# zero-savvy/vimz

Measured on AMD Instinct MI355X. Metric: nova_folding_steps_per_sec, higher is better.
Workload: dtype u32 limbs (256-bit Montgomery integers over BN254 Fr/Fq)

## Files before the change

vimz_amd/csrc/capi.hip:

```cpp
#include <hip/hip_runtime.h>
#include <mutex>
#include <new>
#include <string>
#include <cstring>
#include <cstdio>

#include "internal.hpp"
#define HIP_TRY(c, x) do { hipError_t _e = (x); if (_e != hipSuccess) return vz::vz_fail(c, VIMZ_ERR_HIP, #x, _e); } while (0)
#include "vecops_api.hpp"
#include "ckgen.hpp"

using namespace vz;

static thread_local std::string g_err_noctx;

namespace vz {
int vz_fail(vimz_ctx* c, int code, const char* what, hipError_t e) {
  std::string m = what;
  if (e != hipSuccess) { m += ": "; m += hipGetErrorString(e); }
  static std::mutex err_mu;
  std::lock_guard<std::mutex> g(err_mu);
  if (c) c->err = m; else g_err_noctx = m;
  return code;
}
// ... 601 lines not shown
  uint64_t total = 0;
  for (size_t k = 0; k < blocks; k++) for (size_t g = 0; g < nb; g++) { sum[g] += block_hist[k * nb + g]; total += block_hist[k * nb + g]; }
  if (total >= (1ull << 31)) return fail(c, VIMZ_ERR_INVALID, "vimz_test_msm_scan: more than 2^31 - 1 entries");
  std::lock_guard<std::mutex> g(c->mu);
  HIP_TRY(c, hipSetDevice(c->device));
  TailBufs B;
  uint32_t *hist, *counts, *boff, *soff, *totals, *heavy;
  const size_t heavy_words = 1 + (size_t)MSM_HEAVY_CAP + TAIL_HEAVY_GUARD;
  TAIL_TRY(B.get(&hist, blocks * nb)); TAIL_TRY(B.get(&counts, nb)); TAIL_TRY(B.get(&boff, nb + 1, 0xff)); TAIL_TRY(B.get(&soff, nb + 1, 0xff));
  TAIL_TRY(B.get(&totals, MSM_TOTALS_WORDS, 0)); TAIL_TRY(B.get(&heavy, heavy_words, 0xff));
  for (int call = 0; call < calls; call++) {
    if (lds) {
      TAIL_TRY(tail_up(c, hist, block_hist, blocks * nb));
      launch_prefix_scan(c->stream, hist, (uint32_t)nb, counts, (uint32_t)blocks, heavy, boff, soff, totals, sub, heavy_min, MsmRowStrides(), 1);
    } else {
      TAIL_TRY(tail_up(c, counts, sum.data(), nb));
      TAIL_TRY(hipMemsetAsync(heavy, 0, 4, c->stream));
      launch_scan(c->stream, counts, (uint32_t)nb, boff, soff, totals, sub, heavy, heavy_min);
    }
    TAIL_TRY(hipGetLastError());
    TAIL_TRY(hipStreamSynchronize(c->stream));
  }
  TAIL_TRY(tail_down(c, counts_out, counts, nb)); TAIL_TRY(tail_down(c, bucket_off_out, boff, nb + 1)); TAIL_TRY(tail_down(c, sub_off_out, soff, nb + 1));
  TAIL_TRY(tail_down(c, totals_out, totals, 4)); TAIL_TRY(tail_down(c, heavy_out, heavy, heavy_words));
  if (lds) TAIL_TRY(tail_down(c, block_hist_out, hist, blocks * nb));
  TAIL_TRY(hipStreamSynchronize(c->stream));
  return VIMZ_OK;
}

extern "C" int vimz_test_msm_combine(vimz_ctx* c, int curve, uint32_t* partial, size_t n_slots, const uint32_t* sub_off, size_t nb, const uint32_t* heavy, size_t n_ids, int lane_bits,
                                     uint32_t heavy_min, size_t rows, int calls) {
  if (!c || !partial || !sub_off || !heavy || calls < 1 || !nb || nb >= (1u << 24) || n_slots >= (1u << 24)) return fail(c, VIMZ_ERR_INVALID, "vimz_test_msm_combine: bad argument");
  if (curve < VIMZ_CURVE_BN254_G1 || curve > VIMZ_CURVE_VESTA) return fail(c, VIMZ_ERR_INVALID, "vimz_test_msm_combine: bad curve");
  if (lane_bits < 0 || lane_bits > 4) return fail(c, VIMZ_ERR_INVALID, "vimz_test_msm_combine: lane_bits outside 0..4");
  if (!rows || rows > MSM_ROWS_MAX) return fail(c, VIMZ_ERR_INVALID, "vimz_test_msm_combine: rows outside 1..16");
  if (n_ids > MSM_HEAVY_CAP) return fail(c, VIMZ_ERR_INVALID, "vimz_test_msm_combine: more ids than the heavy list holds");
  for (size_t r = 0; r < rows; r++) {
    const uint32_t* off = sub_off + r * (nb + 1); const uint32_t* hv = heavy + r * (1 + n_ids);
    if (!tail_offsets_ok(off, nb, n_slots)) return fail(c, VIMZ_ERR_INVALID, "vimz_test_msm_combine: sub_off not monotone or outside partial");
    if (hv[0] > MSM_HEAVY_CAP) continue;
    if (hv[0] > n_ids) return fail(c, VIMZ_ERR_INVALID, "vimz_test_msm_combine: the heavy count exceeds the ids given");
    std::vector<bool> seen(nb, false);
    for (uint32_t h = 0; h < hv[0]; h++) {
      const uint32_t b = hv[1 + h];
      if (b >= nb) return fail(c, VIMZ_ERR_INVALID, "vimz_test_msm_combine: a heavy bucket id not below nb");
      if (seen[b] || off[b + 1] - off[b] <= heavy_min) return fail(c, VIMZ_ERR_INVALID, "vimz_test_msm_combine: a heavy bucket listed twice or not above heavy_min");
      seen[b] = true;
    }
  }
  std::lock_guard<std::mutex> g(c->mu);
  HIP_TRY(c, hipSetDevice(c->device));
  const uint32_t G = (uint32_t)rows;
  const MsmRowStrides rs = msm_row_strides(G, 0, (uint32_t)nb, 0, n_slots, 0);
  TailBufs B;
  uint32_t *dp, *doff, *dheavy, *dscr, *ddone;
  TAIL_TRY(B.get(&dp, rows * XYZZ_WORDS * n_slots)); TAIL_TRY(B.get(&doff, rows * (nb + 1))); TAIL_TRY(B.get(&dheavy, rows * ((size_t)MSM_HEAVY_CAP + 1), 0xff));
  TAIL_TRY(B.get(&dscr, rows * MsmWorkspace::HEAVY_SCRATCH_WORDS, 0xff)); TAIL_TRY(B.get(&ddone, rows * (size_t)MSM_HEAVY_DONE_WORDS, 0));
  TAIL_TRY(tail_up(c, doff, sub_off, rows * (nb + 1)));
  for (size_t r = 0; r < rows; r++) TAIL_TRY(tail_up(c, dheavy + r * ((size_t)MSM_HEAVY_CAP + 1), heavy + r * (1 + n_ids), 1 + n_ids));
  const int rc = curve_dispatch(curve, [&](auto cv) {
    typedef typename decltype(cv)::Coord F;
    for (int call = 0; call < calls; call++) {
      TAIL_TRY(tail_up(c, dp, partial, rows * XYZZ_WORDS * n_slots));
      launch_combine<F>(c->stream, dp, doff, (uint32_t)nb, dheavy, dscr, (uint32_t)lane_bits, heavy_min, ddone, rs, G);
      TAIL_TRY(hipGetLastError());
      TAIL_TRY(hipStreamSynchronize(c->stream));
    }
    return (int)VIMZ_OK;
  });
  if (rc) return rc;
  TAIL_TRY(tail_down(c, partial, dp, rows * XYZZ_WORDS * n_slots));
  TAIL_TRY(hipStreamSynchronize(c->stream));
  return VIMZ_OK;
}

extern "C" int vimz_test_msm_reduce(vimz_ctx* c, int curve, const uint32_t* partial, size_t n_slots, const uint32_t* counts, const uint32_t* sub_off, uint32_t nbw, size_t windows,
                                    int mode, size_t rows, int calls, uint32_t* sums_out) {
  if (!c || !partial || !counts || !sub_off || !sums_out || calls < 1 || mode < 0 || mode > 2 || n_slots >= (1u << 24)) return fail(c, VIMZ_ERR_INVALID, "vimz_test_msm_reduce: bad argument");
  if (curve < VIMZ_CURVE_BN254_G1 || curve > VIMZ_CURVE_VESTA) return fail(c, VIMZ_ERR_INVALID, "vimz_test_msm_reduce: bad curve");
  if (nbw < 2 || nbw > 32768 || (nbw & (nbw - 1))) return fail(c, VIMZ_ERR_INVALID, "vimz_test_msm_reduce: nbw not a power of two in 2..32768");
  if (!rows || rows > MSM_ROWS_MAX) return fail(c, VIMZ_ERR_INVALID, "vimz_test_msm_reduce: rows outside 1..16");
  uint32_t Pl = 0, Gp = 0;
  const bool planes_fit = msm_plane_shape(nbw, Pl, Gp);
  if (!windows || windows > (size_t)MSM_MAX_WINDOWS / 2 || (mode == 2 && (windows != 1 || rows != 1 || !planes_fit)))
    return fail(c, VIMZ_ERR_INVALID, "vimz_test_msm_reduce: windows outside 1..48, or bit planes over anything but one row of one bucket set of 1024 buckets or more");
  const size_t nb = (size_t)nbw * windows;
  for (size_t r = 0; r < rows; r++) {
    const uint32_t* off = sub_off + r * (nb + 1);
    if (!tail_offsets_ok(off, nb, n_slots)) return fail(c, VIMZ_ERR_INVALID, "vimz_test_msm_reduce: sub_off not monotone or outside partial");
    for (size_t b = 0; b < nb; b++) if (counts[r * nb + b] && off[b] >= n_slots) return fail(c, VIMZ_ERR_INVALID, "vimz_test_msm_reduce: a filled bucket's slot outside partial");
  }
  std::lock_guard<std::mutex> g(c->mu);
  HIP_TRY(c, hipSetDevice(c->device));
  const uint32_t G = (uint32_t)rows;
  const size_t kout = mode == 2 ? Pl + 2 : mode == 1 ? 2 * windows : windows;
  const MsmRowStrides rs = msm_row_strides(G, 0, (uint32_t)nb, 0, n_slots, (size_t)XYZZ_WORDS * kout);
  TailBufs B;
// ... 315 lines not shown
```

vimz_amd/csrc/ec.hpp:

```cpp
#pragma once
#include "fp.hpp"
#include "fp29.hpp"

namespace vz {

template <class F>
struct Affine { F x, y; };

template <class F>
struct XYZZ {
  F X, Y, ZZ, ZZZ;
  static VZ_HD XYZZ identity() { XYZZ r; r.X = F::zero(); r.Y = F::zero(); r.ZZ = F::zero(); r.ZZZ = F::zero(); return r; }
  VZ_HD bool is_identity() const { return ZZ.is_zero(); }
};

template <class F>
VZ_HD bool aff_is_identity(const Affine<F>& a) { return a.x.is_zero() && a.y.is_zero(); }

template <class F>
VZ_HD XYZZ<F> from_affine(const Affine<F>& a) {
  XYZZ<F> r;
  if (aff_is_identity(a)) return XYZZ<F>::identity();
  r.X = a.x; r.Y = a.y; r.ZZ = F::one(); r.ZZZ = F::one();
  return r;
}


template <class F>
VZ_HD XYZZ<F> dbl_affine(const Affine<F>& a) {
  XYZZ<F> r;
  F U = F::dbl(a.y);
  F V = F::sqr(U);
  F W = F::mul(U, V);
  F S = F::mul(a.x, V);
  F X2 = F::sqr(a.x);
  F M = F::add(F::dbl(X2), X2);
  r.X = F::template sub<4>(F::sqr(M), F::dbl(S));
  r.Y = F::template sub<2>(F::mul(M, F::template sub<6>(S, r.X)), F::mul(W, a.y));
  r.ZZ = V; r.ZZZ = W;
  return r;
}

template <class F>
VZ_HD XYZZ<F> dbl(const XYZZ<F>& p) {
  if (p.is_identity()) return p;
  XYZZ<F> r;
  F U = F::dbl(p.Y);
  F V = F::sqr(U);
  F W = F::mul(U, V);
  F S = F::mul(p.X, V);
  F X2 = F::sqr(p.X);
  F M = F::add(F::dbl(X2), X2);
  r.X = F::template sub<4>(F::sqr(M), F::dbl(S));
  r.Y = F::template sub<2>(F::mul(M, F::template sub<6>(S, r.X)), F::mul(W, p.Y));
  r.ZZ = F::mul(V, p.ZZ);
  r.ZZZ = F::mul(W, p.ZZZ);
  return r;
}

template <int K, class F>
VZ_HD F diff_of_products(const F& a, const F& b, const F& c, const F& d) {
  if constexpr (F::LAZY) return F::mul_add2(a, b, F::template sub<K>(F::zero(), c), d);
  else return F::template sub<2>(F::mul(a, b), F::mul(c, d));
}

template <class F>
VZ_HD void add_mixed(XYZZ<F>& acc, const Affine<F>& q) {
  if (aff_is_identity(q)) return;
  if (acc.is_identity()) { acc.X = q.x; acc.Y = q.y; acc.ZZ = F::one(); acc.ZZZ = F::one(); return; }
  F U2 = F::mul(q.x, acc.ZZ);
  F S2 = F::mul(q.y, acc.ZZZ);
  F Pv = F::template sub<6>(U2, acc.X);
  F R = F::template sub<4>(S2, acc.Y);
  if (Pv.is_zero_mod()) {
    if (R.is_zero_mod()) acc = dbl_affine(q); else acc = XYZZ<F>::identity();
    return;
  }
  F PP = F::sqr(Pv);
  F PPP = F::mul(Pv, PP);
  F Q = F::mul(acc.X, PP);
  F X3 = F::template sub<4>(F::sqr(R), F::add(PPP, F::dbl(Q)));
  F Y3 = diff_of_products<4>(R, F::template sub<6>(Q, X3), acc.Y, PPP);
  acc.X = X3; acc.Y = Y3;
  acc.ZZ = F::mul(acc.ZZ, PP);
  acc.ZZZ = F::mul(acc.ZZZ, PPP);
}

template <class F>
VZ_HD void add_full(XYZZ<F>& acc, const XYZZ<F>& q) {
  if (q.is_identity()) return;
  if (acc.is_identity()) { acc = q; return; }
  F U1 = F::mul(acc.X, q.ZZ);
  F U2 = F::mul(q.X, acc.ZZ);
  F S1 = F::mul(acc.Y, q.ZZZ);
  F S2 = F::mul(q.Y, acc.ZZZ);
  F Pv = F::template sub<2>(U2, U1);
  F R = F::template sub<2>(S2, S1);
  if (Pv.is_zero_mod()) {
    if (R.is_zero_mod()) acc = dbl(acc); else acc = XYZZ<F>::identity();
    return;
  }
  F PP = F::sqr(Pv);
  F PPP = F::mul(Pv, PP);
  F Q = F::mul(U1, PP);
  F X3 = F::template sub<4>(F::sqr(R), F::add(PPP, F::dbl(Q)));
  F Y3 = diff_of_products<2>(R, F::template sub<6>(Q, X3), S1, PPP);
  acc.X = X3; acc.Y = Y3;
  acc.ZZ = F::mul(F::mul(acc.ZZ, q.ZZ), PP);
  acc.ZZZ = F::mul(F::mul(acc.ZZZ, q.ZZZ), PPP);
}

template <class F>
VZ_HD Affine<F> to_affine(const XYZZ<F>& p) {
  Affine<F> a;
  if (p.is_identity()) { a.x = F::zero(); a.y = F::zero(); return a; }
  F zi3 = F::pow_pm2(p.ZZZ);
  F zi2 = F::sqr(F::mul(zi3, p.ZZ));
  a.x = F::mul(p.X, zi2).canon();
// ... 31 lines not shown
```

vimz_amd/csrc/msm.hpp:

```cpp
#pragma once
#include <cstdlib>
#include <cstring>
#include <mutex>
#include "msm_api.hpp"
#include "ec_mem.hpp"

namespace vz {

inline const MsmTuning& msm_tuning() {
  static const MsmTuning t = [] {
    MsmTuning r;
    if (const char* e = getenv("VIMZ_TUNE")) {
      if (const char* q = strstr(e, "sort_blocks=")) r.sort_blocks = atoi(q + 12);
      if (const char* q = strstr(e, "combine_lane_bits=")) r.combine_lane_bits = atoi(q + 18);
      if (const char* q = strstr(e, "ones_dense=")) r.ones_dense = atoi(q + 11);
      if (const char* q = strstr(e, "reduce_planes=")) r.reduce_planes = atoi(q + 14);
      if (const char* q = strstr(e, "signed_scalars=")) r.signed_scalars = atoi(q + 15) != 0;
    }
    return r;
  }();
  return t;
}


__device__ __forceinline__ uint32_t window_bits(const uint32_t* s, int lo, int c) {
  int limb = lo >> 5, off = lo & 31;
  if (limb >= 8) return 0;
  uint64_t v = s[limb];
  if (limb + 1 < 8) v |= (uint64_t)s[limb + 1] << 32;
  return (uint32_t)(v >> off) & ((1u << c) - 1);
}

template <class S>
__device__ __forceinline__ bool load_scalar(const uint32_t* __restrict__ scalars, size_t i, int mont, int skip_ones, int sgn, uint32_t* s, uint32_t& flip) {
  const uint4* p = reinterpret_cast<const uint4*>(scalars + 8 * i);
  uint4 a = p[0], b = p[1];
  S x;
  x.v[0] = a.x; x.v[1] = a.y; x.v[2] = a.z; x.v[3] = a.w; x.v[4] = b.x; x.v[5] = b.y; x.v[6] = b.z; x.v[7] = b.w;
  if (x.is_zero()) return false;
  if (skip_ones) {
    bool one;
    if (mont) one = x.eq(S::one());
    else { uint32_t o = x.v[0] ^ 1u; for (int k = 1; k < 8; k++) o |= x.v[k]; one = o == 0; }
    if (one) return false;
  }
  if (mont) x = S::from_mont(x);
  flip = 0;
  if (sgn) {
    uint32_t t[8]; uint64_t br = 0, lt = 0;
#pragma unroll
// ... 167 lines not shown
  const uint32_t* mine = block_hist + (size_t)blockIdx.x * nb;
  for (uint32_t g = threadIdx.x; g < nb; g += SORT_THREADS) lds_pos[g] = bucket_off[g] + mine[g];
  __syncthreads();
  const size_t chunk = (n + gridDim.x - 1) / gridDim.x;
  const size_t lo = blockIdx.x * chunk, hi = lo + chunk < n ? lo + chunk : n;
  for (size_t i = lo + threadIdx.x; i < hi; i += SORT_THREADS) {
    uint32_t s[8], flip;
    if (!load_scalar<S>(scalars, i, mont, skip_ones, sgn, s, flip)) continue;
    for_each_digit(s, c, K, flip, [&](int w, uint32_t b, uint32_t neg) {
      const uint32_t pos = atomicAdd(&lds_pos[(uint32_t)w * nbw + b], 1u);
      sorted[pos] = ((uint32_t)i + (uint32_t)w * pt_stride) | (neg << 31);
    });
  }
}

template <class F>
__global__ void __launch_bounds__(256, 3) k_accum(const uint32_t* __restrict__ bases, const uint32_t* __restrict__ sorted,
                                               const uint32_t* __restrict__ bucket_off, const uint32_t* __restrict__ sub_off,
                                               uint32_t nb, const uint32_t* __restrict__ totals,
                                               uint32_t* __restrict__ partial, uint32_t sub, MsmRowStrides rs) {
  { const size_t row = blockIdx.y; sorted += row * rs.sorted; bucket_off += row * rs.offs; sub_off += row * rs.offs; totals += row * rs.totals; partial += row * rs.partial; }
  const uint32_t total = totals[0];
  uint32_t s = blockIdx.x * blockDim.x + threadIdx.x;
  if (s >= total) return;
  uint32_t lo = 0, hi = nb;
  while (hi - lo > 1) {
    uint32_t mid = (lo + hi) >> 1;
    if (sub_off[mid] <= s) lo = mid; else hi = mid;
  }
  const uint32_t b = lo, k = s - sub_off[b];
  const uint32_t beg = bucket_off[b] + k * sub;
  const uint32_t end = min(bucket_off[b + 1], beg + sub);
  XYZZ<F> acc = XYZZ<F>::identity();
  uint32_t ent = beg < end ? sorted[beg] : 0u;
  RawAffine raw = load_affine_raw(bases, ent & 0x7fffffffu);
  for (uint32_t e = beg; e < end; e++) {
    const uint32_t ent_n = e + 1 < end ? sorted[e + 1] : ent;
    const RawAffine raw_n = load_affine_raw(bases, ent_n & 0x7fffffffu);
    Affine<F> q = affine_of_raw<F>(raw);
    if ((ent >> 31) && !aff_is_identity(q)) q.y = F::neg(q.y);
    add_mixed(acc, q);
    ent = ent_n; raw = raw_n;
  }
  store_xyzz(partial, s, acc);
}

constexpr uint32_t ONES_THREADS = 16384;
template <class S>
__device__ __forceinline__ bool scalar_is_one(const uint32_t* __restrict__ scalars, size_t i, int mont) {
  const uint4* p = reinterpret_cast<const uint4*>(scalars + 8 * i);
  const uint4 a = p[0], b = p[1];
  if (mont) return a.x == S::Params::R1.w[0] && a.y == S::Params::R1.w[1] && a.z == S::Params::R1.w[2] && a.w == S::Params::R1.w[3] &&
                   b.x == S::Params::R1.w[4] && b.y == S::Params::R1.w[5] && b.z == S::Params::R1.w[6] && b.w == S::Params::R1.w[7];
  return a.x == 1u && (a.y | a.z | a.w | b.x | b.y | b.z | b.w) == 0u;
}
template <class S, class F>
__global__ void __launch_bounds__(256) k_ones_partial(const uint32_t* __restrict__ scalars, const uint32_t* __restrict__ bases, size_t n, int mont,
                                                      uint32_t* __restrict__ out ) {
  const uint32_t t = blockIdx.x * blockDim.x + threadIdx.x;
  XYZZ<F> acc = XYZZ<F>::identity();
  for (size_t i = t; i < n; i += ONES_THREADS)
    if (scalar_is_one<S>(scalars, i, mont)) { Affine<F> q = load_affine<F>(bases, (uint32_t)i); add_mixed(acc, q); }
  store_xyzz(out, t, acc);
}
template <class S, class F>
__device__ __forceinline__ XYZZ<F> ones_dense_sum(const uint32_t* __restrict__ scalars, const uint32_t* __restrict__ bases, size_t n, int mont, uint32_t (*queue)[128]) {
  const uint32_t t = blockIdx.x * blockDim.x + threadIdx.x, lane = threadIdx.x & 63u, wv = threadIdx.x >> 6;
  const size_t wave = t >> 6, nwaves = ONES_THREADS / 64;
  volatile uint32_t* q = queue[wv];
  XYZZ<F> acc = XYZZ<F>::identity();
  uint32_t cnt = 0;
  for (size_t base = wave * 64; base < n; base += nwaves * 64) {
    const size_t i = base + lane;
    const bool one = i < n && scalar_is_one<S>(scalars, i, mont);
    const uint64_t m = __ballot(one);
    if (one) q[cnt + (uint32_t)__popcll(m & ((1ull << lane) - 1ull))] = (uint32_t)i;
    cnt += (uint32_t)__popcll(m);
    __builtin_amdgcn_wave_barrier();
    if (cnt >= 64) {
      cnt -= 64;
      const uint32_t idx = q[cnt + lane];
      __builtin_amdgcn_wave_barrier();
      Affine<F> pt = load_affine<F>(bases, idx);
      add_mixed(acc, pt);
    }
  }
  if (lane < cnt) { Affine<F> pt = load_affine<F>(bases, q[lane]); add_mixed(acc, pt); }
  return acc;
}
template <class S, class F>
__global__ void __launch_bounds__(256) k_ones_dense(const uint32_t* __restrict__ scalars, const uint32_t* __restrict__ bases, size_t n, int mont,
                                                    uint32_t* __restrict__ out ) {
  __shared__ uint32_t queue[4][128];
  const XYZZ<F> acc = ones_dense_sum<S, F>(scalars, bases, n, mont, queue);
  store_xyzz(out, blockIdx.x * blockDim.x + threadIdx.x, acc);
}
template <class S, class F>
__global__ void __launch_bounds__(256) k_ones_dense_rows(OnesDescs ds, int mont, uint32_t* __restrict__ lvl ) {
  __shared__ uint32_t queue[4][128];
  __shared__ XYZZ<F> sh[256];
  const OnesDesc& d = ds.d[blockIdx.y];
  sh[threadIdx.x] = ones_dense_sum<S, F>(d.scalars, d.bases, d.n, mont, queue);
  __syncthreads();
  quad_tree256<F>(sh);
  if (threadIdx.x == 0) store_xyzz(lvl, (size_t)blockIdx.y * gridDim.x + blockIdx.x, sh[0]);
}
template <class F>
__global__ void __launch_bounds__(256) k_tree_rows(const uint32_t* __restrict__ lvl, uint32_t m , OnesDescs ds) {
  __shared__ XYZZ<F> sh[256];
  const uint32_t t = threadIdx.x;
  sh[t] = t < m ? load_xyzz<F>(lvl, (size_t)blockIdx.x * m + t) : XYZZ<F>::identity();
  __syncthreads();
  quad_tree256<F>(sh);
  if (t == 0) store_xyzz(ds.d[blockIdx.x].out, 0, sh[0]);
}
template <class F>
__global__ void __launch_bounds__(256) k_tree256(const uint32_t* __restrict__ in, uint32_t m, uint32_t* __restrict__ out) {
  __shared__ XYZZ<F> sh[256];
  const uint32_t t = threadIdx.x, i = blockIdx.x * 256 + t;
  sh[t] = i < m ? load_xyzz<F>(in, i) : XYZZ<F>::identity();
  __syncthreads();
  quad_tree256<F>(sh);
  if (t == 0) store_xyzz(out, blockIdx.x, sh[0]);
}


constexpr uint32_t MSM_HEAVY_PARTS = 32, MSM_HEAVY_SPLIT = 1024;
constexpr uint32_t MSM_HEAVY_SPLIT_MIN = 2048;
constexpr uint32_t COMBINE_HEAVY_BLOCKS = 512, COMBINE_SPLIT_BLOCKS = 1024;

template <class F>
__global__ void __launch_bounds__(256) k_combine(uint32_t* __restrict__ partial, const uint32_t* __restrict__ sub_off, uint32_t nb, uint32_t nbn,
                                                 const uint32_t* __restrict__ heavy, uint32_t heavy_cap, uint32_t* scratch ,
                                                 uint32_t lane_bits , uint32_t heavy_min,
                                                 uint32_t* __restrict__ heavy_done , MsmRowStrides rs) {
  __shared__ XYZZ<F> sh[256];
  __shared__ uint32_t s_last;
  const uint32_t t = threadIdx.x;
  { const size_t row = blockIdx.y; partial += row * rs.partial; sub_off += row * rs.offs; heavy += row * rs.heavy; scratch += row * rs.heavy_scratch; heavy_done += row * rs.heavy_done; }
  if (blockIdx.x < nbn) {
    const uint32_t L = 1u << lane_bits, lane = t & (L - 1u);
    const uint32_t b = blockIdx.x * (256u >> lane_bits) + (t >> lane_bits);
    uint32_t s0 = 0, m = 0;
    if (b < nb) { s0 = sub_off[b]; m = sub_off[b + 1] - s0; }
    if (m > heavy_min && heavy[0] <= heavy_cap) m = 0;
    if (!__syncthreads_or(m >= 2 ? 1 : 0)) return;
    XYZZ<F> acc = XYZZ<F>::identity();
    if (lane < m) acc = load_xyzz<F>(partial, s0 + lane);
    for (uint32_t k = lane + L; k < m; k += L) { XYZZ<F> q = load_xyzz<F>(partial, s0 + k); add_full(acc, q); }
    sh[t] = acc;
    __syncthreads();
    for (uint32_t d = L >> 1; d > 0; d >>= 1) {
      if (lane < d && lane + d < m) { XYZZ<F> a = sh[t]; add_full(a, sh[t + d]); sh[t] = a; }
      __syncthreads();
    }
    if (lane == 0 && m >= 2) store_xyzz(partial, s0, sh[t]);
    return;
  }
  const uint32_t count = heavy[0] <= heavy_cap ? heavy[0] : 0u;
  if (blockIdx.x < nbn + COMBINE_HEAVY_BLOCKS) {
    for (uint32_t h = blockIdx.x - nbn; h < count; h += COMBINE_HEAVY_BLOCKS) {
      const uint32_t b = heavy[1 + h];
      const uint32_t s0 = sub_off[b], m = sub_off[b + 1] - s0;
      if (h < MSM_HEAVY_SPLIT && m >= MSM_HEAVY_SPLIT_MIN) continue;
      XYZZ<F> acc = XYZZ<F>::identity();
      for (uint32_t k = t; k < m; k += 256) { XYZZ<F> q = load_xyzz<F>(partial, s0 + k); add_full(acc, q); }
      __syncthreads();
      sh[t] = acc;
      __syncthreads();
      quad_tree256<F>(sh);
      if (t == 0) store_xyzz(partial, s0, sh[0]);
    }
// ... 164 lines not shown
        if (dig[k]) atomicAdd(&cnt[(dig[k] < 0 ? -dig[k] : dig[k]) - 1], 1u);
      }
    }
  }
  __syncthreads();
  if (t < 64) {
    const uint32_t c0 = cnt[t];
    uint32_t m4 = (c0 + 3) / 4, m5 = (c0 + 4) / 5, m6 = (c0 + 5) / 6, m7 = (c0 + 6) / 7;
    for (int o = 32; o > 0; o >>= 1) { m4 += __shfl_xor(m4, o); m5 += __shfl_xor(m5, o); m6 += __shfl_xor(m6, o); m7 += __shfl_xor(m7, o); }
    const uint32_t sub = m4 <= SMALL_THREADS ? 4u : m5 <= SMALL_THREADS ? 5u : m6 <= SMALL_THREADS ? 6u : m7 <= SMALL_THREADS ? 7u : 8u;
    const uint32_t m = (c0 + sub - 1) / sub;
    uint32_t ic = c0, im = m, mx = m;
    for (int o = 1; o < 64; o <<= 1) {
      const uint32_t uc = __shfl_up(ic, o), um = __shfl_up(im, o);
      if ((int)t >= o) { ic += uc; im += um; }
    }
    for (int o = 32; o > 0; o >>= 1) mx = max(mx, (uint32_t)__shfl_xor(mx, o));
    off[t] = ic - c0; soff[t] = im - m;
    if (t == 63) { off[SMALL_NBW] = ic; soff[SMALL_NBW] = im; s_maxm = mx; }
  }
  __syncthreads();
#pragma unroll
  for (int k = 0; k < (int)SMALL_PER_THREAD; k++) {
    if (dig[k]) {
      const uint32_t b = (uint32_t)(dig[k] < 0 ? -dig[k] : dig[k]) - 1;
      const uint32_t pos = atomicAdd(&cur[b], 1u);
      list[off[b] + pos] = (uint16_t)((t + SMALL_THREADS * k) | (dig[k] < 0 ? 0x8000u : 0u));
    }
  }
  if (t < SMALL_NBW) for (uint32_t sb = soff[t]; sb < soff[t + 1]; sb++) subb[sb] = (uint8_t)t;
  __syncthreads();
  const uint32_t nsubs = soff[SMALL_NBW];
  XYZZ<F> acc = XYZZ<F>::identity();
  uint32_t kk = 0, mb = 0;
  if (t < nsubs) {
    const uint32_t b = subb[t];
    kk = t - soff[b]; mb = soff[b + 1] - soff[b];
    const uint32_t cb = off[b + 1] - off[b];
    const uint32_t beg = off[b] + kk * cb / mb, end = off[b] + (kk + 1) * cb / mb;
    uint32_t ent = beg < end ? list[beg] : 0u;
    Affine<F> pt = load_affine<F>(wbases, lo + (ent & 0x7fffu));
    for (uint32_t e = beg; e < end; e++) {
      const uint32_t ent_n = e + 1 < end ? list[e + 1] : ent;
      const Affine<F> pt_n = load_affine<F>(wbases, lo + (ent_n & 0x7fffu));
      if ((ent & 0x8000u) && !aff_is_identity(pt)) pt.y = F::neg(pt.y);
      add_mixed(acc, pt);
      ent = ent_n; pt = pt_n;
    }
  }
  sh[t] = acc;
  __syncthreads();
  for (uint32_t d = 1; d < s_maxm; d <<= 1) {
    const bool act = t < nsubs && (kk & (2 * d - 1)) == 0 && kk + d < mb;
    const uint64_t bal = __ballot(act);
    if ((t & 63) == 0) wcnt[t >> 6] = (uint32_t)__popcll(bal);
    __syncthreads();
    uint32_t before = 0, total = 0;
    for (uint32_t wv = 0; wv < SMALL_THREADS / 64; wv++) { before += wv < (t >> 6) ? wcnt[wv] : 0u; total += wcnt[wv]; }
    if (act) list[before + (uint32_t)__popcll(bal & ((1ull << (t & 63)) - 1ull))] = (uint16_t)t;
    __syncthreads();
    for (uint32_t base = 0; base < total; base += 64)
      quad_level<F>(sh, min(64u, total - base), [&](uint32_t e) { return (uint32_t)list[base + e]; }, [&](uint32_t e) { return (uint32_t)list[base + e] + d; });
  }
  XYZZ<F> bk = XYZZ<F>::identity();
  if (t < SMALL_NBW && cnt[t]) bk = sh[soff[t]];
  __syncthreads();
  if (Q > 1 && done) {
    if (t < SMALL_NBW) {
      store_xyzz(chunk_out, ((size_t)w * Q + q) * SMALL_NBW + t, bk);
      __threadfence();
      if (t == 0) s_ticket = atomicAdd(&done[w], 1u);
    }
    __syncthreads();
    if (s_ticket != Q - 1) return;
    __threadfence();

    const uint32_t b = t & (SMALL_NBW - 1), sl = t / SMALL_NBW;
    for (uint32_t loaded = 0; loaded < Q;) {
      const uint32_t slot0 = loaded ? 1u : 0u, k = min(Q - loaded, 4u - slot0), m = slot0 + k;
// ... 138 lines not shown
    for (int k = 0; k < c; k++) acc = dbl(acc);
    p = to_affine(acc);
    store_affine<F>(tables, (size_t)j * n + i, p);
  }
}
template <class C>
hipError_t build_tables(hipStream_t stream, const uint32_t* d_bases, size_t n, int c, int K, uint32_t* d_tables) {
  typedef typename C::Coord F;
  if (!n) return hipSuccess;
  hipLaunchKernelGGL(k_build_tables<F>, dim3((unsigned)((n + 255) / 256)), dim3(256), 0, stream, d_bases, n, c, K, d_tables);
  return hipGetLastError();
}

static inline MsmRowStrides msm_row_strides(uint32_t G, size_t scalar_words, uint32_t nb, size_t entries, size_t max_subs, size_t out_words) {
  MsmRowStrides rs;
  if (G > 1) {
    rs.scalars = scalar_words; rs.block_hist = (size_t)SORT_BLOCKS * nb; rs.sorted = entries; rs.partial = (size_t)XYZZ_WORDS * max_subs;
    rs.heavy_scratch = MsmWorkspace::HEAVY_SCRATCH_WORDS; rs.out = out_words;
    rs.counts = nb; rs.offs = nb + 1; rs.totals = MSM_TOTALS_WORDS; rs.heavy = MSM_HEAVY_CAP + 1; rs.heavy_done = MSM_HEAVY_DONE_WORDS;
  }
  return rs;
}
static inline void launch_prefix_scan(hipStream_t stream, uint32_t* block_hist, uint32_t nb, uint32_t* counts, uint32_t sort_blocks, uint32_t* heavy, uint32_t* bucket_off,
                                      uint32_t* sub_off, uint32_t* totals, uint32_t sub, uint32_t heavy_min, const MsmRowStrides& rs, uint32_t G) {
  hipLaunchKernelGGL(k_prefix_scan<0>, dim3((nb + 1023) / 1024, G), dim3(1024), 0, stream, block_hist, nb, counts, sort_blocks, heavy, bucket_off, sub_off,
                     totals, sub, heavy_min, MSM_HEAVY_CAP, rs);
}
static inline void launch_scan(hipStream_t stream, const uint32_t* counts, uint32_t nb, uint32_t* bucket_off, uint32_t* sub_off, uint32_t* totals, uint32_t sub, uint32_t* heavy,
                               uint32_t heavy_min) {
  hipLaunchKernelGGL(k_scan<MSM_SUB>, dim3(1), dim3(1024), 0, stream, counts, nb, bucket_off, sub_off, totals, sub, heavy, heavy_min, MSM_HEAVY_CAP);
}
template <class F>
static void launch_combine(hipStream_t stream, uint32_t* partial, const uint32_t* sub_off, uint32_t nb, const uint32_t* heavy, uint32_t* heavy_scratch, uint32_t lane_bits,
                           uint32_t heavy_min, uint32_t* heavy_done, const MsmRowStrides& rs, uint32_t G) {
  const unsigned per_wg = 256u >> lane_bits, nbn = (nb + per_wg - 1) / per_wg;
  hipLaunchKernelGGL(k_combine<F>, dim3(nbn + COMBINE_HEAVY_BLOCKS + COMBINE_SPLIT_BLOCKS, G), dim3(256), 0, stream, partial, sub_off, nb, nbn,
                     heavy, MSM_HEAVY_CAP, heavy_scratch, lane_bits, heavy_min, heavy_done, rs);
}
template <class F>
static void launch_reduce(hipStream_t stream, const uint32_t* partial, const uint32_t* counts, const uint32_t* sub_off, uint32_t nbw, uint32_t windows, uint32_t* window_sums,
                          uint32_t* plain_sums, const MsmRowStrides& rs, uint32_t G) {
  hipLaunchKernelGGL(k_reduce<F>, dim3(windows, G), dim3(nbw < 256 ? nbw : 256), 0, stream, partial, counts, sub_off, nbw, window_sums, plain_sums, rs);
}
template <class F>
static void launch_reduce_planes(hipStream_t stream, const uint32_t* partial, const uint32_t* counts, const uint32_t* sub_off, uint32_t nbw, uint32_t Pl, uint32_t Gp,
                                 uint32_t* plane_scratch, uint32_t* ticket, uint32_t* out) {
  hipLaunchKernelGGL(k_reduce_planes<F>, dim3((Pl + 2) * Gp), dim3(256), 0, stream, partial, counts, sub_off, nbw, Pl, Gp, nbw / (512u * Gp), plane_scratch, ticket, out);
}
template <class F>
static void launch_accum(hipStream_t stream, const uint32_t* bases, const uint32_t* sorted, const uint32_t* bucket_off, const uint32_t* sub_off, uint32_t nb, const uint32_t* totals,
                         uint32_t* partial, uint32_t sub, size_t max_subs, const MsmRowStrides& rs, uint32_t G) {
  hipLaunchKernelGGL(k_accum<F>, dim3((unsigned)((max_subs + 255) / 256), G), dim3(256), 0, stream, bases, sorted, bucket_off, sub_off, nb, totals, partial, sub, rs);
}
template <class S, class F>
static void launch_ones(hipStream_t stream, bool dense, const uint32_t* scalars, const uint32_t* bases, size_t n, int mont, uint32_t* lvl0) {
  if (dense) hipLaunchKernelGGL((k_ones_dense<S, F>), dim3(ONES_THREADS / 256), dim3(256), 0, stream, scalars, bases, n, mont, lvl0);
  else hipLaunchKernelGGL((k_ones_partial<S, F>), dim3(ONES_THREADS / 256), dim3(256), 0, stream, scalars, bases, n, mont, lvl0);
}
template <class F>
static void launch_tree256(hipStream_t stream, const uint32_t* in, uint32_t m, uint32_t* tmp, uint32_t* out) {
  if (m > 256) {
    hipLaunchKernelGGL(k_tree256<F>, dim3((m + 255) / 256), dim3(256), 0, stream, in, m, tmp);
    in = tmp; m = (m + 255) / 256;
  }
  hipLaunchKernelGGL(k_tree256<F>, dim3(1), dim3(256), 0, stream, in, m, out);
}
template <class F>
static void launch_tree_rows(hipStream_t stream, const uint32_t* lvl, uint32_t m, const OnesDescs& ds, uint32_t count) {
  hipLaunchKernelGGL(k_tree_rows<F>, dim3(count), dim3(256), 0, stream, lvl, m, ds);
}
// ... 96 lines not shown

template <class C>
static hipError_t launch_unit_sums(const MsmCall& a, const MsmShape& sh, uint32_t G) {
  typedef typename C::Coord F;
  typedef typename C::Scalar S;
  const MsmRowGroup* rg = a.rg;
  if (rg) {
    OnesDesc ds[2 * MSM_ROWS_MAX];
    for (uint32_t r = 0; r < G; r++) ds[r] = OnesDesc{a.d_scalars + 8 * r * rg->scalar_row_stride, a.d_bases, a.wsum + r * (rg->pinned_row_stride / 4) + (size_t)XYZZ_WORDS * sh.kout, a.n};
    for (uint32_t e = 0; e < rg->n_extra; e++) ds[G + e] = rg->extra[e];
    return ones_launch_rows<C>(a.stream, a.ws, ds, G + rg->n_extra, a.scalars_mont);
  }
  uint32_t* lvl0 = reinterpret_cast<uint32_t*>(a.ws.ones_partial);
  launch_ones<S, F>(a.stream, msm_tuning().ones_dense != 0, a.d_scalars, a.d_bases, a.n, a.scalars_mont, lvl0);
  uint32_t* lvl1 = lvl0 + (size_t)XYZZ_WORDS * ONES_THREADS;
  launch_tree256<F>(a.stream, lvl0, ONES_THREADS, lvl1, a.wsum + (size_t)XYZZ_WORDS * sh.kout);
  return hipSuccess;
}

template <class C>
static hipError_t launch_large(const MsmCall& a, const MsmShape& sh) {
  typedef typename C::Coord F;
  typedef typename C::Scalar S;
  const MsmPlan& pl = sh.plan;
  const MsmRowGroup* rg = a.rg;
  MsmWorkspace& ws = a.ws;
  const uint32_t G = rg ? rg->G : 1u;
  VZ_HIP_CHECK(ws.reserve(pl.nb, sh.entries, sh.max_subs, rg ? std::max<size_t>(G, rg->max_rows) : 1));
  const MsmRowStrides rs = msm_row_strides(G, rg ? 8 * rg->scalar_row_stride : 0, pl.nb, sh.entries, sh.max_subs, rg ? rg->pinned_row_stride / 4 : 0);
  VZ_HIP_CHECK(launch_sort<S>(a, sh, rs, G));
  uint32_t* partial = reinterpret_cast<uint32_t*>(ws.partial);
  launch_accum<F>(a.stream, a.d_bases, ws.sorted, ws.bucket_off, ws.sub_off, pl.nb, ws.totals, partial, sh.sub, sh.max_subs, rs, G);
  VZ_EV(4);
  launch_combine<F>(a.stream, partial, ws.sub_off, pl.nb, ws.heavy, ws.heavy_scratch, sh.lane_bits, sh.heavy_min, ws.heavy_done, rs, G);
  VZ_EV(5);
  if (sh.planes) launch_reduce_planes<F>(a.stream, partial, ws.counts, ws.sub_off, pl.nbw, sh.Pl, sh.Gp, ws.plane_scratch, ws.totals + 3, a.wsum);
  else if (sh.shared) launch_reduce<F>(a.stream, partial, ws.counts, ws.sub_off, sh.vw, (uint32_t)sh.V, a.wsum, a.wsum + (size_t)XYZZ_WORDS * sh.V, rs, G);
  else launch_reduce<F>(a.stream, partial, ws.counts, ws.sub_off, pl.nbw, (uint32_t)pl.K, a.wsum, nullptr, rs, G);
  VZ_EV(6);
  if (a.split_ones) VZ_HIP_CHECK(launch_unit_sums<C>(a, sh, G));
  return hipGetLastError();
}
#undef VZ_EV

template <class C>
static hipError_t msm_launch_impl(hipStream_t stream, MsmWorkspace& ws, const uint32_t* d_bases, const uint32_t* d_scalars, size_t n,
                                  int scalars_mont, int c_override, void* pinned_dst, MsmPlan* plan_out, hipEvent_t* ev, int split_ones,
                                  const BaseTables* tb, const MsmRowGroup* rg) {
  MsmShape sh;
  MsmGroupDesc gd;
  if (rg) { gd.grouped = true; gd.G = rg->G; gd.n_extra = rg->n_extra; }
  const int rc = msm_shape(sh, n, C::Scalar::Params::BITS, c_override, split_ones, msm_table_desc(tb), gd, msm_tuning(), msm_no_small());
  if (rc != MSM_SHAPE_OK) return rc == MSM_SHAPE_NOT_SUPPORTED ? hipErrorNotSupported : hipErrorInvalidValue;
  *plan_out = sh.plan;
  if (sh.path == MSM_PATH_LARGE && sh.plan.tabled) d_bases = tb->d + (size_t)AFFINE_WORDS * tb->offset;
  const MsmCall a{stream, ws, d_bases, d_scalars, n, scalars_mont, msm_tuning().signed_scalars, split_ones, reinterpret_cast<uint32_t*>(pinned_dst), ev, tb, rg};
  switch (sh.path) {
    case MSM_PATH_FIXED: return launch_fixed<C>(a, sh);
    case MSM_PATH_SMALL: return launch_small<C>(a, sh, msm_small_sum_kernel());
    default: return launch_large<C>(a, sh);
  }
}

template <class C>
hipError_t msm_launch(hipStream_t stream, MsmWorkspace& ws, const uint32_t* d_bases, const uint32_t* d_scalars, size_t n,
                      int scalars_mont, int c_override, void* pinned_dst, MsmPlan* plan_out, hipEvent_t* ev, int split_ones,
                      const BaseTables* tb) {
// ... 113 lines not shown
```

vimz_amd/csrc/msm_shape.hpp:

```cpp
#pragma once
#include <cstdint>
#include <cstddef>
#include <algorithm>

namespace vz {

constexpr int MSM_SUB = 16;
constexpr int MSM_MAX_WINDOWS = 96;
constexpr uint32_t MSM_VWIN = 1024;
constexpr uint32_t MSM_ROWS_MAX = 16;

struct MsmPlan {
  int c;
  int K;
  uint32_t nbw;
  uint32_t nb;
  int split_ones;
  int tabled;
};

constexpr int SMALL_C = 7;
constexpr uint32_t SMALL_CHUNK = 1536, SMALL_MAXQ = 32;
constexpr uint32_t SMALL_NBW = 1u << (SMALL_C - 1);
constexpr size_t MSM_SMALL_MAX = (size_t)SMALL_CHUNK * 20;
static_assert(MSM_SMALL_MAX <= (size_t)SMALL_CHUNK * SMALL_MAXQ, "chunk results of a window fit the workspace");
constexpr uint32_t FIXED_PER_THREAD = 4, FIXED_CHUNK = 256 * FIXED_PER_THREAD;
constexpr uint32_t SORT_BLOCKS = 256;
constexpr uint32_t MSM_TOTALS_WORDS = 16, MSM_HEAVY_CAP = 65536, MSM_HEAVY_DONE_WORDS = 1024;
constexpr uint32_t MSM_HEAVY_SCRATCH_POINTS = 1024 * 32;

static inline MsmPlan msm_plan(size_t n, int scalar_bits, int c_override) {
  MsmPlan p;
  p.split_ones = 0; p.tabled = 0;
  int c = c_override;
  if (c <= 0) {
    c = n >= (1u << 15) ? 11 : n >= (1u << 12) ? 9 : n >= 256 ? 7 : 5;
  }
  p.c = c;
  p.K = (scalar_bits + 1 + c - 1) / c;
  p.nbw = 1u << (c - 1);
  p.nb = p.nbw * (uint32_t)p.K;
  return p;
}

static inline uint32_t msm_vwin(const MsmPlan& p) { return std::min<uint32_t>(p.nbw, MSM_VWIN); }
static inline int msm_vwindows(const MsmPlan& p) { return (int)(p.nbw / msm_vwin(p)); }
static inline uint32_t msm_plane_bits(const MsmPlan& p) { uint32_t P = 0; while ((1u << P) < p.nbw) P++; return P; }
static inline bool msm_plane_shape(uint32_t nbw, uint32_t& Pl, uint32_t& Gp) {
  Pl = 0; while ((1u << Pl) < nbw) Pl++;
  Gp = std::min<uint32_t>(16u, nbw / 1024u);
  while (Gp > 1 && (Pl + 2) * Gp > 256) Gp >>= 1;
  return nbw >= 1024 && (1u << Pl) == nbw && (Pl + 2) * Gp <= 256 && (int)Pl + 2 + 1 <= MSM_MAX_WINDOWS;
}
static inline int msm_kout(const MsmPlan& p) { return p.tabled == 4 ? (int)msm_plane_bits(p) + 2 : p.tabled == 1 ? 2 * msm_vwindows(p) : p.K; }
static inline int msm_sums_out(const MsmPlan& p) { return msm_kout(p) + (p.split_ones ? 1 : 0); }

struct MsmTuning { int sort_blocks = 0, combine_lane_bits = -1, ones_dense = 1, reduce_planes = 0, signed_scalars = 1; };
struct MsmTableDesc { bool present = false; int c = 0, K = 0, own = 0; bool mult = false; size_t n_total = 0; };
struct MsmGroupDesc { bool grouped = false; uint32_t G = 1, n_extra = 0; };

enum MsmPath { MSM_PATH_FIXED, MSM_PATH_SMALL, MSM_PATH_LARGE };
enum { MSM_SHAPE_OK = 0, MSM_SHAPE_INVALID = 1, MSM_SHAPE_NOT_SUPPORTED = 2  };

struct MsmShape {
  MsmPath path = MSM_PATH_LARGE;
  MsmPlan plan = {};
  uint32_t Q = 0, chunk = 0, Qf = 0;
  bool lds_sort = false;
  bool own = false;
  bool shared = false;
  bool planes = false;
  uint32_t sub = 0;
  size_t entries = 0, max_subs = 0;
  uint32_t sort_blocks = 0, lane_bits = 0, heavy_min = 0;
  uint32_t bstride = 0 , pstride = 0 ;
  uint32_t vw = 0; int V = 0;
  uint32_t Pl = 0, Gp = 0;
  int kout = 0;
};

static inline int msm_shape(MsmShape& out, size_t n, int scalar_bits, int c_override, int split_ones, const MsmTableDesc& tb, const MsmGroupDesc& rg,
                            const MsmTuning& tune, bool no_small) {
  MsmShape s;
  if (n == 0 || n >= (1u << 31)) return MSM_SHAPE_INVALID;
  if (rg.grouped && (rg.G == 0 || rg.G > MSM_ROWS_MAX || rg.n_extra > MSM_ROWS_MAX || (split_ones == 0 && rg.n_extra))) return MSM_SHAPE_INVALID;
  const bool small_fmt = tb.present && tb.c == SMALL_C;
  const bool small_tb = small_fmt && !no_small && c_override <= 0;
  bool tabled = tb.present && !small_fmt && c_override <= 0;
  if (tabled && tb.own && tb.c != msm_plan(n, scalar_bits, 0).c) tabled = false;
  s.own = tabled && tb.own;
  s.shared = tabled && !tb.own;
  if (small_tb && (n > MSM_SMALL_MAX || tb.K != (scalar_bits + SMALL_C) / SMALL_C)) return MSM_SHAPE_INVALID;
  if (!no_small && !tabled && c_override <= 0 && n <= MSM_SMALL_MAX) {
    if (rg.grouped) return MSM_SHAPE_NOT_SUPPORTED;
    MsmPlan& ps = s.plan;
    ps.c = SMALL_C; ps.K = (scalar_bits + SMALL_C) / SMALL_C; ps.nbw = SMALL_NBW; ps.nb = SMALL_NBW * (uint32_t)ps.K; ps.split_ones = 0; ps.tabled = small_tb ? 2 : 0;
    s.kout = msm_kout(ps);
    if (small_tb && tb.mult) {
      s.path = MSM_PATH_FIXED;
      s.Qf = (uint32_t)((n + FIXED_CHUNK - 1) / FIXED_CHUNK);
    } else {
      s.path = MSM_PATH_SMALL;
      s.Q = (uint32_t)((n + SMALL_CHUNK - 1) / SMALL_CHUNK); s.chunk = (uint32_t)((n + s.Q - 1) / s.Q);
    }
    out = s;
    return MSM_SHAPE_OK;
  }
  s.path = MSM_PATH_LARGE;
  MsmPlan& pl = s.plan;
  pl = msm_plan(n, scalar_bits, tabled ? tb.c : c_override);
  if (tabled) {
    if (tb.K != pl.K || pl.nbw < 256 || (size_t)tb.K * tb.n_total >= (1u << 31)) return MSM_SHAPE_INVALID;
    if (!s.own && 2 * msm_vwindows(pl) + 1 > MSM_MAX_WINDOWS) return MSM_SHAPE_INVALID;
    if (s.own) pl.tabled = 3; else { pl.nb = pl.nbw; pl.tabled = 1; }
  }
  if (pl.K + 1 > MSM_MAX_WINDOWS || pl.c > 16 || pl.c < 2) return MSM_SHAPE_INVALID;
  pl.split_ones = split_ones;
  const bool planes_fit = msm_plane_shape(pl.nbw, s.Pl, s.Gp);
  s.planes = s.shared && tune.reduce_planes && planes_fit;
  if (s.planes) pl.tabled = 4;
  s.lds_sort = (size_t)pl.nb * 4 <= 144 * 1024;
  if (rg.grouped && (s.planes || s.own || !s.lds_sort)) return MSM_SHAPE_NOT_SUPPORTED;
  s.entries = (size_t)pl.K * n;
  s.sub = n < (1u << 15) ? 8u : split_ones ? (n < (1u << 19) ? 8u : (uint32_t)MSM_SUB) : (uint32_t)MSM_SUB;
  s.max_subs = s.entries / s.sub + pl.nb + 1;
  s.sort_blocks = tune.sort_blocks > 0 && tune.sort_blocks <= (int)SORT_BLOCKS ? (uint32_t)tune.sort_blocks
                                                                                 : (uint32_t)std::min<size_t>(SORT_BLOCKS, std::max<size_t>(32, n / 4096));
  s.bstride = s.shared ? 0u : pl.nbw; s.pstride = tabled ? (uint32_t)tb.n_total : 0u;
  const size_t mean_parts = (split_ones ? s.entries / 8 : s.entries) / s.sub / pl.nb + 1;
  s.lane_bits = tune.combine_lane_bits >= 0 ? (uint32_t)tune.combine_lane_bits : mean_parts > 96 ? 4u : mean_parts > 48 ? 3u : mean_parts > 24 ? 2u : 1u;
  s.heavy_min = 16u << s.lane_bits;
  s.vw = msm_vwin(pl); s.V = msm_vwindows(pl); s.kout = msm_kout(pl);
  out = s;
  return MSM_SHAPE_OK;
}

}
```

Before: 1430.

## Add packed slot-parallel MSM combine and cheaper first mixed addition

Adds a packed combine mode that assigns one thread per partial-sum slot across all buckets and runs a workgroup tree reduction in LDS with compacted pair lists. The old mode mapped a fixed number of lanes to each bucket. The packed mode is on by default when heavy_min is at most 32, and it is meant to avoid idle lanes when buckets hold few partials. Separately, the first mixed addition after an affine load now skips the ZZ/ZZZ multiplies (add_mixed_first), and dbl_affine gains a y==0 identity check. The costs are a larger shared-memory array, which may lower occupancy, and extra barriers per reduction level.

```diff
diff --git a/vimz_amd/csrc/capi.hip b/vimz_amd/csrc/capi.hip
--- a/vimz_amd/csrc/capi.hip
+++ b/vimz_amd/csrc/capi.hip
@@ -657,6 +657,8 @@
                                      uint32_t heavy_min, size_t rows, int calls) {
   if (!c || !partial || !sub_off || !heavy || calls < 1 || !nb || nb >= (1u << 24) || n_slots >= (1u << 24)) return fail(c, VIMZ_ERR_INVALID, "vimz_test_msm_combine: bad argument");
   if (curve < VIMZ_CURVE_BN254_G1 || curve > VIMZ_CURVE_VESTA) return fail(c, VIMZ_ERR_INVALID, "vimz_test_msm_combine: bad curve");
+  const bool packed = lane_bits >= 0 && (lane_bits & 0x100) != 0;
+  if (packed) lane_bits &= 0xff;
   if (lane_bits < 0 || lane_bits > 4) return fail(c, VIMZ_ERR_INVALID, "vimz_test_msm_combine: lane_bits outside 0..4");
   if (!rows || rows > MSM_ROWS_MAX) return fail(c, VIMZ_ERR_INVALID, "vimz_test_msm_combine: rows outside 1..16");
   if (n_ids > MSM_HEAVY_CAP) return fail(c, VIMZ_ERR_INVALID, "vimz_test_msm_combine: more ids than the heavy list holds");
@@ -687,7 +689,7 @@
     typedef typename decltype(cv)::Coord F;
     for (int call = 0; call < calls; call++) {
       TAIL_TRY(tail_up(c, dp, partial, rows * XYZZ_WORDS * n_slots));
-      launch_combine<F>(c->stream, dp, doff, (uint32_t)nb, dheavy, dscr, (uint32_t)lane_bits, heavy_min, ddone, rs, G);
+      launch_combine<F>(c->stream, dp, doff, (uint32_t)nb, dheavy, dscr, (uint32_t)lane_bits, heavy_min, ddone, rs, G, packed, n_slots);
       TAIL_TRY(hipGetLastError());
       TAIL_TRY(hipStreamSynchronize(c->stream));
     }
diff --git a/vimz_amd/csrc/ec.hpp b/vimz_amd/csrc/ec.hpp
--- a/vimz_amd/csrc/ec.hpp
+++ b/vimz_amd/csrc/ec.hpp
@@ -28,6 +28,7 @@
 
 template <class F>
 VZ_HD XYZZ<F> dbl_affine(const Affine<F>& a) {
+  if (a.y.is_zero_mod()) return XYZZ<F>::identity();
   XYZZ<F> r;
   F U = F::dbl(a.y);
   F V = F::sqr(U);
@@ -84,6 +85,34 @@
   acc.X = X3; acc.Y = Y3;
   acc.ZZ = F::mul(acc.ZZ, PP);
   acc.ZZZ = F::mul(acc.ZZZ, PPP);
+}
+
+template <class F>
+VZ_HD void add_mixed_first(XYZZ<F>& acc, const Affine<F>& q) {
+  if (aff_is_identity(q)) return;
+  if (acc.is_identity()) { acc.X = q.x; acc.Y = q.y; acc.ZZ = F::one(); acc.ZZZ = F::one(); return; }
+  F Pv = F::template sub<2>(q.x, acc.X);
+  F R = F::template sub<2>(q.y, acc.Y);
+  if (Pv.is_zero_mod()) {
+    if (R.is_zero_mod()) acc = dbl_affine(q); else acc = XYZZ<F>::identity();
+    return;
+  }
+  F PP = F::sqr(Pv);
+  F PPP = F::mul(Pv, PP);
+  F Q = F::mul(acc.X, PP);
+  F X3 = F::template sub<4>(F::sqr(R), F::add(PPP, F::dbl(Q)));
+  F Y3 = diff_of_products<2>(R, F::template sub<6>(Q, X3), acc.Y, PPP);
+  acc.X = X3; acc.Y = Y3;
+  acc.ZZ = PP;
+  acc.ZZZ = PPP;
+}
+
+template <class F>
+VZ_HD void add_mixed_chain(XYZZ<F>& acc, bool& plain, const Affine<F>& q) {
+  if (aff_is_identity(q)) return;
+  if (acc.is_identity()) { acc.X = q.x; acc.Y = q.y; acc.ZZ = F::one(); acc.ZZZ = F::one(); plain = true; return; }
+  if (plain) { add_mixed_first(acc, q); plain = false; }
+  else add_mixed(acc, q);
 }
 
 template <class F>
diff --git a/vimz_amd/csrc/msm.hpp b/vimz_amd/csrc/msm.hpp
--- a/vimz_amd/csrc/msm.hpp
+++ b/vimz_amd/csrc/msm.hpp
@@ -16,6 +16,7 @@
       if (const char* q = strstr(e, "ones_dense=")) r.ones_dense = atoi(q + 11);
       if (const char* q = strstr(e, "reduce_planes=")) r.reduce_planes = atoi(q + 14);
       if (const char* q = strstr(e, "signed_scalars=")) r.signed_scalars = atoi(q + 15) != 0;
+      if (const char* q = strstr(e, "combine_packed=")) r.combine_packed = atoi(q + 15) != 0;
     }
     return r;
   }();
@@ -249,6 +250,7 @@
   const uint32_t beg = bucket_off[b] + k * sub;
   const uint32_t end = min(bucket_off[b + 1], beg + sub);
   XYZZ<F> acc = XYZZ<F>::identity();
+  bool plain = false;
   uint32_t ent = beg < end ? sorted[beg] : 0u;
   RawAffine raw = load_affine_raw(bases, ent & 0x7fffffffu);
   for (uint32_t e = beg; e < end; e++) {
@@ -256,7 +258,7 @@
     const RawAffine raw_n = load_affine_raw(bases, ent_n & 0x7fffffffu);
     Affine<F> q = affine_of_raw<F>(raw);
     if ((ent >> 31) && !aff_is_identity(q)) q.y = F::neg(q.y);
-    add_mixed(acc, q);
+    add_mixed_chain(acc, plain, q);
     ent = ent_n; raw = raw_n;
   }
   store_xyzz(partial, s, acc);
@@ -276,8 +278,9 @@
                                                       uint32_t* __restrict__ out ) {
   const uint32_t t = blockIdx.x * blockDim.x + threadIdx.x;
   XYZZ<F> acc = XYZZ<F>::identity();
+  bool plain = false;
   for (size_t i = t; i < n; i += ONES_THREADS)
-    if (scalar_is_one<S>(scalars, i, mont)) { Affine<F> q = load_affine<F>(bases, (uint32_t)i); add_mixed(acc, q); }
+    if (scalar_is_one<S>(scalars, i, mont)) { Affine<F> q = load_affine<F>(bases, (uint32_t)i); add_mixed_chain(acc, plain, q); }
   store_xyzz(out, t, acc);
 }
 template <class S, class F>
@@ -286,6 +289,7 @@
   const size_t wave = t >> 6, nwaves = ONES_THREADS / 64;
   volatile uint32_t* q = queue[wv];
   XYZZ<F> acc = XYZZ<F>::identity();
+  bool plain = false;
   uint32_t cnt = 0;
   for (size_t base = wave * 64; base < n; base += nwaves * 64) {
     const size_t i = base + lane;
@@ -299,10 +303,10 @@
       const uint32_t idx = q[cnt + lane];
       __builtin_amdgcn_wave_barrier();
       Affine<F> pt = load_affine<F>(bases, idx);
-      add_mixed(acc, pt);
-    }
-  }
-  if (lane < cnt) { Affine<F> pt = load_affine<F>(bases, q[lane]); add_mixed(acc, pt); }
+      add_mixed_chain(acc, plain, pt);
+    }
+  }
+  if (lane < cnt) { Affine<F> pt = load_affine<F>(bases, q[lane]); add_mixed_chain(acc, plain, pt); }
   return acc;
 }
 template <class S, class F>
@@ -346,15 +350,77 @@
 constexpr uint32_t MSM_HEAVY_SPLIT_MIN = 2048;
 constexpr uint32_t COMBINE_HEAVY_BLOCKS = 512, COMBINE_SPLIT_BLOCKS = 1024;
 
+constexpr uint32_t COMBINE_PACKED_SLOTS = 256 + COMBINE_PACKED_HEAVY_MAX - 1;
+constexpr uint32_t COMBINE_WAVES = 256 / 64;
+template <class F>
+__device__ __forceinline__ void combine_packed_wg(XYZZ<F>* __restrict__ sh , uint32_t* __restrict__ partial, const uint32_t* __restrict__ sub_off,
+                                                  uint32_t nb, bool listed , uint32_t heavy_min) {
+  __shared__ uint32_t s_tail[2], wcnt[COMBINE_WAVES + 1];
+  __shared__ uint16_t pairs[COMBINE_PACKED_SLOTS / 2 + 1];
+  const uint32_t t = threadIdx.x, first = blockIdx.x * 256u, total = sub_off[nb];
+  if (first >= total) return;
+  const uint32_t hm = min(heavy_min, COMBINE_PACKED_HEAVY_MAX);
+  uint32_t s0 = 0, m0 = 0, k0 = 0, mser = 0;
+  if (first + t < total) {
+    const uint32_t s = first + t;
+    uint32_t lo = 0, hi = nb;
+    while (hi - lo > 1) {
+      const uint32_t mid = (lo + hi) >> 1;
+      if (sub_off[mid] <= s) lo = mid; else hi = mid;
+    }
+    s0 = sub_off[lo];
+    const uint32_t m = sub_off[lo + 1] - s0;
+    k0 = s - s0;
+    if (s0 >= first && m >= 2 && !(listed && m > heavy_min)) {
+      if (m <= hm) m0 = m; else if (k0 == 0) mser = m;
+    }
+  }
+  if (!__syncthreads_or((m0 | mser) ? 1 : 0)) return;
+  if (t == min(255u, total - 1u - first)) { s_tail[0] = m0 ? s0 : 0u; s_tail[1] = m0 ? s0 + m0 : 0u; }
+  __syncthreads();
+  uint32_t m1 = 0, k1 = 0;
+  if (first + 256u + t < s_tail[1]) { m1 = s_tail[1] - s_tail[0]; k1 = first + 256u + t - s_tail[0]; }
+  if (m0) sh[t] = load_xyzz<F>(partial, first + t);
+  if (m1) sh[256u + t] = load_xyzz<F>(partial, first + 256u + t);
+  if (mser) {
+    XYZZ<F> acc = load_xyzz<F>(partial, s0);
+    for (uint32_t k = 1; k < mser; k++) { XYZZ<F> q = load_xyzz<F>(partial, s0 + k); add_full(acc, q); }
+    store_xyzz(partial, s0, acc);
+  }
+  __syncthreads();
+  const uint32_t lane = t & 63u, wv = t >> 6;
+  for (uint32_t d = 1; d < hm; d <<= 1) {
+    const bool a0 = m0 && (k0 & (2 * d - 1)) == 0 && k0 + d < m0, a1 = m1 && (k1 & (2 * d - 1)) == 0 && k1 + d < m1;
+    const uint64_t b0 = __ballot(a0), b1 = __ballot(a1);
+    if (lane == 0) { wcnt[wv] = (uint32_t)__popcll(b0); if (wv == 0) wcnt[COMBINE_WAVES] = (uint32_t)__popcll(b1); }
+    __syncthreads();
+    uint32_t before = 0, n0 = 0;
+    for (uint32_t w = 0; w < COMBINE_WAVES; w++) { before += w < wv ? wcnt[w] : 0u; n0 += wcnt[w]; }
+    const uint32_t npairs = n0 + wcnt[COMBINE_WAVES];
+    if (!npairs) break;
+    const uint64_t below = (1ull << lane) - 1ull;
+    if (a0) pairs[before + (uint32_t)__popcll(b0 & below)] = (uint16_t)t;
+    if (a1) pairs[n0 + (uint32_t)__popcll(b1 & below)] = (uint16_t)(256u + t);
+    __syncthreads();
+    if (t < npairs) { const uint32_t ia = pairs[t]; XYZZ<F> a = sh[ia]; add_full(a, sh[ia + d]); sh[ia] = a; }
+    __syncthreads();
+  }
+  if (m0 && k0 == 0) store_xyzz(partial, s0, sh[t]);
+}
+
 template <class F>
 __global__ void __launch_bounds__(256) k_combine(uint32_t* __restrict__ partial, const uint32_t* __restrict__ sub_off, uint32_t nb, uint32_t nbn,
                                                  const uint32_t* __restrict__ heavy, uint32_t heavy_cap, uint32_t* scratch ,
                                                  uint32_t lane_bits , uint32_t heavy_min,
-                                                 uint32_t* __restrict__ heavy_done , MsmRowStrides rs) {
-  __shared__ XYZZ<F> sh[256];
+                                                 uint32_t* __restrict__ heavy_done , MsmRowStrides rs, uint32_t packed) {
+  __shared__ XYZZ<F> sh[COMBINE_PACKED_SLOTS];
   __shared__ uint32_t s_last;
   const uint32_t t = threadIdx.x;
   { const size_t row = blockIdx.y; partial += row * rs.partial; sub_off += row * rs.offs; heavy += row * rs.heavy; scratch += row * rs.heavy_scratch; heavy_done += row * rs.heavy_done; }
+  if (blockIdx.x < nbn && packed) {
+    combine_packed_wg<F>(sh, partial, sub_off, nb, heavy[0] <= heavy_cap, heavy_min);
+    return;
+  }
   if (blockIdx.x < nbn) {
     const uint32_t L = 1u << lane_bits, lane = t & (L - 1u);
     const uint32_t b = blockIdx.x * (256u >> lane_bits) + (t >> lane_bits);
@@ -585,6 +651,7 @@
   __syncthreads();
   const uint32_t nsubs = soff[SMALL_NBW];
   XYZZ<F> acc = XYZZ<F>::identity();
+  bool plain = false;
   uint32_t kk = 0, mb = 0;
   if (t < nsubs) {
     const uint32_t b = subb[t];
@@ -597,7 +664,7 @@
       const uint32_t ent_n = e + 1 < end ? list[e + 1] : ent;
       const Affine<F> pt_n = load_affine<F>(wbases, lo + (ent_n & 0x7fffu));
       if ((ent & 0x8000u) && !aff_is_identity(pt)) pt.y = F::neg(pt.y);
-      add_mixed(acc, pt);
+      add_mixed_chain(acc, plain, pt);
       ent = ent_n; pt = pt_n;
     }
   }
@@ -802,10 +869,10 @@
 }
 template <class F>
 static void launch_combine(hipStream_t stream, uint32_t* partial, const uint32_t* sub_off, uint32_t nb, const uint32_t* heavy, uint32_t* heavy_scratch, uint32_t lane_bits,
-                           uint32_t heavy_min, uint32_t* heavy_done, const MsmRowStrides& rs, uint32_t G) {
-  const unsigned per_wg = 256u >> lane_bits, nbn = (nb + per_wg - 1) / per_wg;
+                           uint32_t heavy_min, uint32_t* heavy_done, const MsmRowStrides& rs, uint32_t G, bool packed = false, size_t max_subs = 0) {
+  const unsigned per_wg = 256u >> lane_bits, nbn = packed ? (unsigned)((max_subs + 255) / 256) : (nb + per_wg - 1) / per_wg;
   hipLaunchKernelGGL(k_combine<F>, dim3(nbn + COMBINE_HEAVY_BLOCKS + COMBINE_SPLIT_BLOCKS, G), dim3(256), 0, stream, partial, sub_off, nb, nbn,
-                     heavy, MSM_HEAVY_CAP, heavy_scratch, lane_bits, heavy_min, heavy_done, rs);
+                     heavy, MSM_HEAVY_CAP, heavy_scratch, lane_bits, heavy_min, heavy_done, rs, packed ? 1u : 0u);
 }
 template <class F>
 static void launch_reduce(hipStream_t stream, const uint32_t* partial, const uint32_t* counts, const uint32_t* sub_off, uint32_t nbw, uint32_t windows, uint32_t* window_sums,
@@ -968,7 +1035,7 @@
   uint32_t* partial = reinterpret_cast<uint32_t*>(ws.partial);
   launch_accum<F>(a.stream, a.d_bases, ws.sorted, ws.bucket_off, ws.sub_off, pl.nb, ws.totals, partial, sh.sub, sh.max_subs, rs, G);
   VZ_EV(4);
-  launch_combine<F>(a.stream, partial, ws.sub_off, pl.nb, ws.heavy, ws.heavy_scratch, sh.lane_bits, sh.heavy_min, ws.heavy_done, rs, G);
+  launch_combine<F>(a.stream, partial, ws.sub_off, pl.nb, ws.heavy, ws.heavy_scratch, sh.lane_bits, sh.heavy_min, ws.heavy_done, rs, G, sh.combine_packed, sh.max_subs);
   VZ_EV(5);
   if (sh.planes) launch_reduce_planes<F>(a.stream, partial, ws.counts, ws.sub_off, pl.nbw, sh.Pl, sh.Gp, ws.plane_scratch, ws.totals + 3, a.wsum);
   else if (sh.shared) launch_reduce<F>(a.stream, partial, ws.counts, ws.sub_off, sh.vw, (uint32_t)sh.V, a.wsum, a.wsum + (size_t)XYZZ_WORDS * sh.V, rs, G);
diff --git a/vimz_amd/csrc/msm_shape.hpp b/vimz_amd/csrc/msm_shape.hpp
--- a/vimz_amd/csrc/msm_shape.hpp
+++ b/vimz_amd/csrc/msm_shape.hpp
@@ -28,6 +28,7 @@
 constexpr uint32_t SORT_BLOCKS = 256;
 constexpr uint32_t MSM_TOTALS_WORDS = 16, MSM_HEAVY_CAP = 65536, MSM_HEAVY_DONE_WORDS = 1024;
 constexpr uint32_t MSM_HEAVY_SCRATCH_POINTS = 1024 * 32;
+constexpr uint32_t COMBINE_PACKED_HEAVY_MAX = 32;
 
 static inline MsmPlan msm_plan(size_t n, int scalar_bits, int c_override) {
   MsmPlan p;
@@ -55,7 +56,7 @@
 static inline int msm_kout(const MsmPlan& p) { return p.tabled == 4 ? (int)msm_plane_bits(p) + 2 : p.tabled == 1 ? 2 * msm_vwindows(p) : p.K; }
 static inline int msm_sums_out(const MsmPlan& p) { return msm_kout(p) + (p.split_ones ? 1 : 0); }
 
-struct MsmTuning { int sort_blocks = 0, combine_lane_bits = -1, ones_dense = 1, reduce_planes = 0, signed_scalars = 1; };
+struct MsmTuning { int sort_blocks = 0, combine_lane_bits = -1, ones_dense = 1, reduce_planes = 0, signed_scalars = 1, combine_packed = 1; };
 struct MsmTableDesc { bool present = false; int c = 0, K = 0, own = 0; bool mult = false; size_t n_total = 0; };
 struct MsmGroupDesc { bool grouped = false; uint32_t G = 1, n_extra = 0; };
 
@@ -73,6 +74,7 @@
   uint32_t sub = 0;
   size_t entries = 0, max_subs = 0;
   uint32_t sort_blocks = 0, lane_bits = 0, heavy_min = 0;
+  bool combine_packed = false;
   uint32_t bstride = 0 , pstride = 0 ;
   uint32_t vw = 0; int V = 0;
   uint32_t Pl = 0, Gp = 0;
@@ -130,6 +132,7 @@
   const size_t mean_parts = (split_ones ? s.entries / 8 : s.entries) / s.sub / pl.nb + 1;
   s.lane_bits = tune.combine_lane_bits >= 0 ? (uint32_t)tune.combine_lane_bits : mean_parts > 96 ? 4u : mean_parts > 48 ? 3u : mean_parts > 24 ? 2u : 1u;
   s.heavy_min = 16u << s.lane_bits;
+  s.combine_packed = tune.combine_packed != 0 && s.heavy_min <= COMBINE_PACKED_HEAVY_MAX;
   s.vw = msm_vwin(pl); s.V = msm_vwindows(pl); s.kout = msm_kout(pl);
   out = s;
   return MSM_SHAPE_OK;
```

Result: slower. 1409 (-1.4%).
